# muzishen/IMAGDressing

Hardware: AMD Instinct MI355X
Metric: 512x512 50-step images/sec (whole node) (higher is better)
Workload: dtype bf16

## Files before the change

imagdressing_amd/csrc/conv_gemm.hip:

```cpp
#include "gemm_common.h"

namespace {

template <int BM, int BN, int BK, int WAVES_M> struct TileCfg {
    static constexpr int STRIDE = BK * 2 + 16;
    static constexpr int MAIN = 2 * (BM + BN) * STRIDE;
    static constexpr int CLD = BN + 4;
    static constexpr int EROWS = BM / WAVES_M;
    static constexpr int EPI = EROWS * CLD * 4;
    static constexpr int LDS = MAIN > EPI ? MAIN : EPI;
};

template <bool F16, int BM, int BN, int BK, int WAVES_M, int WAVES_N, int DEPTH>
__global__ __launch_bounds__(WAVES_M * WAVES_N * 64, (WAVES_M * WAVES_N == 4) ? 2 : 1) void conv_gemm_kernel(const ConvGemmParams p) {
    constexpr int NT = WAVES_M * WAVES_N * 64;
    using E = El<F16>;
    using T = TileCfg<BM, BN, BK, WAVES_M>;
    constexpr int TM = BM / WAVES_M / 32;
    constexpr int TN = BN / WAVES_N / 32;
    constexpr int STRIDE = T::STRIDE;
    constexpr int VPR = BK / 8;
    constexpr int RSTEP = NT / VPR;
    constexpr int A_VECS = BM / RSTEP;
    constexpr int W_VECS = BN / RSTEP;
// ... 461 lines not shown
        const int nparts = splitk_stats_parts_of(p);
        if (nparts == 0) return imd_set_error("%s: gn_stats_out on a K-sliced problem that cannot produce the statistics", what);
        const int HW = p.Hout * p.Wout, B = p.M / HW, rpp = fs_rows_per_part(B, HW, p.N);
        if (h) hipLaunchKernelGGL(splitk_finish_stats_kernel<true>, dim3((unsigned)nparts, (unsigned)B), dim3(FS_THREADS), 0, s, p, rpp, nparts);
        else hipLaunchKernelGGL(splitk_finish_stats_kernel<false>, dim3((unsigned)nparts, (unsigned)B), dim3(FS_THREADS), 0, s, p, rpp, nparts);
        return imd_check_launch(what);
    }
    const long chunks = (long)p.M * ((p.N + 7) / 8);
    long blocks = (chunks + 255) / 256;
    if (blocks > 2048) blocks = 2048;
    if (h) hipLaunchKernelGGL(splitk_finish_kernel<true>, dim3((unsigned)blocks), dim3(256), 0, s, p);
    else hipLaunchKernelGGL(splitk_finish_kernel<false>, dim3((unsigned)blocks), dim3(256), 0, s, p);
    return imd_check_launch(what);
}

template <bool F16, int BM, int BN, int BK, int WM, int WN, int DEPTH = 2>
int launch_cfg(const ConvGemmParams& p, hipStream_t s) {
    static_assert(DEPTH == 2 || DEPTH == 4, "pipeline depth");
    constexpr int lds = TileCfg<BM, BN, BK, WM>::LDS;
    auto kern = conv_gemm_kernel<F16, BM, BN, BK, WM, WN, DEPTH>;
    if (int rc_attr = imd_lds_attr(reinterpret_cast<const void*>(kern), lds, "conv_gemm")) return rc_attr;
    const long mt = (p.M + BM - 1) / BM, nt = (p.N + BN - 1) / BN;
    hipLaunchKernelGGL(kern, dim3((unsigned)(mt * nt), (unsigned)p.split_k), dim3(WM * WN * 64), lds, s, p);
    int rc = imd_check_launch("conv_gemm");
    if (rc || p.split_k <= 1 || p.splitk_counters != nullptr) return rc;
    return launch_splitk_finish(p, s, "conv_gemm split-K finish");
}

int tile_dims(int cfg, int* bm, int* bn) {
    switch (cfg) {
        case 0: *bm = 128; *bn = 128; return 0;
        case 1: *bm = 128; *bn = 64; return 0;
        case 2: *bm = 64; *bn = 64; return 0;
        case 4: case 5: case 8: case 29: *bm = 128; *bn = 128; return 0;
        case 3: case 7: *bm = 64; *bn = 64; return 0;
        case 6: *bm = 64; *bn = 320; return 0;
        case 9: case 21: case 30: case 31: *bm = 256; *bn = 128; return 0;
        case 32: *bm = 192; *bn = 128; return 0;
        case 22: *bm = 128; *bn = 160; return 0;
        case 23: *bm = 256; *bn = 160; return 0;
        case 24: *bm = 512; *bn = 64; return 0;
        case 10: case 16: *bm = 256; *bn = 256; return 0;
        case 17: case 18: case 19: case 20: case 25: case 26: case 27: case 28: *bm = 128; *bn = 128; return 0;
        case 11: *bm = 128; *bn = 320; return 0;
        default: return 1;
    }
}

}

int g_gemm_flags = 23;

int imd_gemm_pick_order(const ConvGemmParams& p, int n_tiles) {
    const double a_bytes = (double)p.x_bytes, w_bytes = (double)p.w_bytes / (p.split_k > 1 ? p.split_k : 1);
    const double a_split = a_bytes / (p.split_k > 1 && p.taps == 1 ? p.split_k : 1);
    const double cost_m = a_split + 8.0 * w_bytes;
    const double cost_n = (n_tiles < 8 ? n_tiles : 8) * a_split + w_bytes;
    return cost_m <= cost_n ? 4 : 8;
}

int imd_conv_gemm_stats_parts_of(const ConvGemmParams& p_in, int cfg) {
    ConvGemmParams p = p_in;
    if (p.split_k < 1) p.split_k = 1;
    if (cfg < 0) cfg = imd_conv_gemm_choose_cfg(p.M, p.N);
    if (p.split_k > 1) {
        if (cfg == 21 || cfg == 22 || cfg == 23 || cfg == 24 || cfg == 29 || (cfg >= 17 && cfg <= 20) || (cfg >= 25 && cfg <= 28) || (cfg >= 30 && cfg <= 32)) p.splitk_counters = nullptr;
        return splitk_stats_parts_of(p);
    }
    if (cfg == 22 || cfg == 23) return imd_conv_patch3_stats_parts_of(p, cfg == 23 ? 8 : 4);
    if (cfg == 5 || cfg == 29) return imd_conv_patch_stats_parts_of(p);
    if (cfg == 0 || cfg == 1 || cfg == 2 || cfg == 3 || cfg == 4 || cfg == 7) {
        int bm = 0, bn = 0;
        tile_dims(cfg, &bm, &bn);
        const int HW = p.Hout * p.Wout, G = p.gn_stats_groups;
        if (p.out_f32 || p.mode != OUT_ROWMAJOR || p.act == ACT_GEGLU || G <= 0 || G > 64 || p.N % G || (p.N / G) < 8 || (p.N % 4) || HW <= 0 || HW % bm || p.M % HW) return 0;
        return (HW / bm) * ((p.N + bn - 1) / bn);
    }
    return 0;
}

bool imd_row_linear_gn_in_supported_of(const ConvGemmParams& p, int cfg) {
    if (p.gn_in_partial == nullptr) return true;
    ConvGemmParams q = p;
    q.split_k = 1;
    switch (cfg) {
        case 12: return imd_row_linear_supported(q) && gn_in_ok(q, 320, 128);
        case 13: return imd_row_linear_k640_supported(q) && gn_in_ok(q, 640, 128);
        case 14: return imd_row_linear_k1280_supported(q) && gn_in_ok(q, 1280, 64);
        default: return false;
    }
}

bool imd_conv_gemm_gn_out_supported_of(const ConvGemmParams& p_in, int cfg) {
    ConvGemmParams p = p_in;
    (void)cfg;
    p.splitk_counters = nullptr;
    return splitk_gn_out_supported(p);
}

int imd_conv_gemm_choose_cfg(int M, int N) {
    const long b128 = (long)((M + 127) / 128) * ((N + 127) / 128);
    if (b128 < 96) return 2;
    if (N <= 64) return 1;
// ... 29 lines not shown
    if (p.M <= 0 || p.N <= 0 || p.K <= 0) return imd_set_error("conv_gemm: empty problem M=%d N=%d K=%d", p.M, p.N, p.K);
    if ((p.K % 8) || (p.Cin % 8) || (p.x_pix_stride % 8))
        return imd_set_error("conv_gemm: K (%d), Cin (%d) and pixel stride (%d) must be multiples of 8", p.K, p.Cin, p.x_pix_stride);
    if (p.N % 4) return imd_set_error("conv_gemm: N (%d) must be a multiple of 4", p.N);
    if (p.taps != 1 && p.taps != 9) return imd_set_error("conv_gemm: taps must be 1 or 9 (got %d)", p.taps);
    if (p.K != p.taps * p.Cin) return imd_set_error("conv_gemm: K (%d) != taps*Cin (%d)", p.K, p.taps * p.Cin);
    if (p.mode == OUT_HEADS && (p.hD % 8)) return imd_set_error("conv_gemm: head dim (%d) must be a multiple of 8", p.hD);
    if (p.act == ACT_GEGLU && (p.N % 8)) return imd_set_error("conv_gemm: GEGLU needs N %% 8 == 0");
    if (!imd_conv_gemm_fill_extents(p)) return imd_set_error("conv_gemm: operand larger than 4 GiB");
    if (cfg < 0) cfg = imd_conv_gemm_choose_cfg(p.M, p.N);
    if (p.split_k < 1) p.split_k = 1;
    const unsigned tag = (unsigned)p_in.flags & IMD_TUNING_TAG_MASK;
    if (tag != 0 && tag != (unsigned)IMD_TUNING_PER_CALL)
        return imd_set_error("conv_gemm: flags = 0x%x on entry is neither 0 nor IMD_TUNING_PER_CALL | bits (an uninitialised parameter block?)", (unsigned)p_in.flags);
    const int gf = (tag == (unsigned)IMD_TUNING_PER_CALL) ? ((p_in.flags & 31) | (g_gemm_flags & ~31)) : g_gemm_flags;
    {
        const int bk = (cfg == 4) ? 32 : 64;
        p.flags = 0;
        const bool big_map = p.taps == 9 && p.Wout >= 32;
        if ((gf & 1) && big_map && (p.Cin % bk) == 0) p.flags |= 1;
        if ((gf & 2) && big_map) p.flags |= 2;
    }
    if (gf & 4) {
        int bm = 128, bn = 128;
        tile_dims(cfg, &bm, &bn);
        p.flags |= imd_gemm_pick_order(p, (p.N + bn - 1) / bn);
        p.flags |= gf & 16;
    }
#ifdef IMD_ABLATIONS
    p.flags |= gf & 224;
#endif
    if (p.split_k <= 1) p.splitk_counters = nullptr;
    if (p.gn_stats_out != nullptr && imd_conv_gemm_stats_parts_of(p, cfg) == 0)
        return imd_set_error("conv_gemm: gn_stats_out needs tile config 5 / 22 / 23 / 29 or a register-staged tile (0..4, 7) with H W %% its rows == 0, without K slices, or any K-sliced launch with a separate finish; a row-major 16-bit "
                             "output and 1 <= groups <= 64 with N %% groups == 0 and N / groups >= 8 (got cfg=%d split_k=%d groups=%d N=%d); ask "
                             "imd_conv_gemm_stats_parts() first", cfg, p.split_k, p.gn_stats_groups, p.N);
    if (p.gn_out_gamma != nullptr && !imd_conv_gemm_gn_out_supported_of(p, cfg))
        return imd_set_error("conv_gemm: gn_out_* needs K slices with a separate finish launch, a row-major 16-bit output without residual / activation / scale / "
                             "gn_stats_out, 4 | N / groups and H W N / groups <= %d (got cfg=%d split_k=%d groups=%d N=%d); ask imd_conv_gemm_gn_out_supported() first",
                             4 * FG_THREADS * FG_MAXU, cfg, p.split_k, p.gn_out_groups, p.N);
    if (p.gn_out_gamma != nullptr) p.splitk_counters = nullptr;
    if (p.splitk_counters != nullptr) {
        int bm = 128, bn = 128;
        if (cfg == 5) { bm = 128; bn = 128; } else tile_dims(cfg, &bm, &bn);
        const long tiles = (cfg == 5) ? (long)(p.M / (p.Hout * p.Wout)) * ((p.Hout + 7) / 8) * ((p.Wout + 15) / 16) * ((p.N + 127) / 128)
                                      : (long)((p.M + bm - 1) / bm) * ((p.N + bn - 1) / bn);
        if (tiles > IMD_SPLITK_COUNTERS || (size_t)p.M * p.N * 4 >= 0x80000000ull) p.splitk_counters = nullptr;
    }
    if (p.split_k > 1) {
        if (p.mode == OUT_HEADS || p.act == ACT_GEGLU) return imd_set_error("conv_gemm: split-K supports row-major epilogues only");
        if (!p.splitk_ws) return imd_set_error("conv_gemm: split_k = %d needs a workspace", p.split_k);
    }
    if (p.dtype != IMD_DTYPE_BF16 && p.dtype != IMD_DTYPE_F16) return imd_set_error("conv_gemm: unknown dtype %d", p.dtype);
    if ((p.gn_a != nullptr) != (p.gn_b != nullptr)) return imd_set_error("conv_gemm: gn_a and gn_b must be given together");
    if (p.gn_a != nullptr && cfg != 5) return imd_set_error("conv_gemm: the fused GroupNorm prologue needs tile config 5 (got %d)", cfg);
    if (p.res_rows != 0 && cfg != 12)
        return imd_set_error("conv_gemm: a periodic residual (res_rows = %d) exists in the K = 320 row-resident projection only (tile config 12, got %d)", p.res_rows, cfg);
    if (p.gn_in_partial != nullptr && !imd_row_linear_gn_in_supported_of(p, cfg))
        return imd_set_error("conv_gemm: gn_in_* (GroupNorm of the input rows) exists in the row-resident projections only (tile configs 12 / 13 / 14 with H W a multiple of "
                             "their row block; got cfg=%d K=%d HW=%d): ask imd_row_linear_gn_in_supported() first", cfg, p.K, p.Hout * p.Wout);
    const bool h = p.dtype == IMD_DTYPE_F16;
    switch (cfg) {
        case 0: return h ? launch_cfg<true, 128, 128, 64, 2, 2>(p, s) : launch_cfg<false, 128, 128, 64, 2, 2>(p, s);
        case 1: return h ? launch_cfg<true, 128, 64, 64, 2, 2>(p, s) : launch_cfg<false, 128, 64, 64, 2, 2>(p, s);
        case 2: return h ? launch_cfg<true, 64, 64, 64, 2, 2>(p, s) : launch_cfg<false, 64, 64, 64, 2, 2>(p, s);
        case 3: return h ? launch_cfg<true, 64, 64, 64, 2, 2, 4>(p, s) : launch_cfg<false, 64, 64, 64, 2, 2, 4>(p, s);
        case 4: return h ? launch_cfg<true, 128, 128, 32, 2, 2>(p, s) : launch_cfg<false, 128, 128, 32, 2, 2>(p, s);
        case 6: return h ? launch_cfg<true, 64, 320, 32, 2, 2>(p, s) : launch_cfg<false, 64, 320, 32, 2, 2>(p, s);
        case 7: return h ? launch_cfg<true, 64, 64, 32, 2, 2, 4>(p, s) : launch_cfg<false, 64, 64, 32, 2, 2, 4>(p, s);
        case 8: return h ? launch_cfg<true, 128, 128, 32, 2, 2, 4>(p, s) : launch_cfg<false, 128, 128, 32, 2, 2, 4>(p, s);
        case 9: return h ? launch_cfg<true, 256, 128, 32, 4, 2>(p, s) : launch_cfg<false, 256, 128, 32, 4, 2>(p, s);
        case 10: return h ? launch_cfg<true, 256, 256, 32, 4, 2>(p, s) : launch_cfg<false, 256, 256, 32, 4, 2>(p, s);
        case 11: return h ? launch_cfg<true, 128, 320, 64, 4, 2>(p, s) : launch_cfg<false, 128, 320, 64, 4, 2>(p, s);
        case 5: {
            int rc = imd_launch_conv_patch(p, s);
            if (rc || p.split_k <= 1 || p.splitk_counters != nullptr) return rc;
            return launch_splitk_finish(p, s, "conv_patch split-K finish");
        }
        case 29: {
            p.splitk_counters = nullptr;
            int rc = imd_launch_conv_patch64(p, s);
            if (rc || p.split_k <= 1) return rc;
            return launch_splitk_finish(p, s, "conv_patch split-K finish");
        }
        case 21: {
            p.splitk_counters = nullptr;
            int rc = imd_launch_conv_patch2(p, s);
            if (rc || p.split_k <= 1) return rc;
            return launch_splitk_finish(p, s, "conv_patch2 split-K finish");
        }
        case 22: case 23: {
            int rc = cfg == 22 ? imd_launch_conv_patch3(p, s) : imd_launch_conv_patch4(p, s);
            if (rc || p.split_k <= 1) return rc;
            p.splitk_counters = nullptr;
            return launch_splitk_finish(p, s, "conv_patch3 split-K finish");
        }
        case 25: case 26: case 27: case 28: {
            if ((cfg == 26 || cfg == 28) != (p.taps == 9)) return imd_set_error("conv_gemm: tile config %d does not take taps = %d", cfg, p.taps);
            p.splitk_counters = nullptr;
            int rc = imd_launch_gemm_dma128(p, cfg >= 27 ? 13 : 12, s);
            if (rc || p.split_k <= 1) return rc;
            return launch_splitk_finish(p, s, "gemm_dma128 split-K finish");
        }
        case 24: {
            p.splitk_counters = nullptr;
            if (p.split_k <= 1) return imd_set_error("conv_gemm: tile config 24 writes K-slice slabs only (split_k >= 2)");
            int rc = imd_launch_conv_img(p, s);
            if (rc) return rc;
            return launch_splitk_finish(p, s, "conv_img split-K finish");
        }
        case 30: case 31: case 32: {
// ... 21 lines not shown
```

imagdressing_amd/csrc/conv_patch.hip:

```cpp
#include <type_traits>

#include "gemm_common.h"
#include "lds_dma.h"

namespace {

constexpr int TH = 8, TW = 16;
constexpr int PW = TW + 2, PH = TH + 2;
constexpr int NPIX = PH * PW;
constexpr int CK = 32;
constexpr int RSTR = CK * 2 + 16;
constexpr int BN = 128;
constexpr int A_BYTES = NPIX * RSTR;
constexpr int W_BYTES = BN * RSTR;
constexpr int MAIN_LDS = 2 * A_BYTES + 2 * W_BYTES;
constexpr int CLD = BN + 4;
constexpr int EROWS = 64;
constexpr int EPI_LDS = EROWS * CLD * 4;
constexpr int PATCH_LDS = MAIN_LDS > EPI_LDS ? MAIN_LDS : EPI_LDS;
constexpr int A_VECS = (NPIX * (CK / 8) + 255) / 256;
__device__ constexpr unsigned char kColPix[32] = {0, 1, 2, 3, 8, 9, 10, 11, 12, 13, 14, 15, 4, 5, 6, 7,
                                                  30, 31, 16, 17, 22, 23, 24, 25, 26, 27, 28, 29, 18, 19, 20, 21};
constexpr int W_VECS = BN * (CK / 8) / 256;

constexpr int AB_D = 12 * 1024, WB_D = 8 * 1024, NWR_D = 3;
constexpr int PATCH_DMA_LDS = 2 * AB_D + NWR_D * WB_D;
static_assert(PATCH_DMA_LDS >= EPI_LDS, "the epilogue tile must fit the main-loop LDS");
template <int CKD> struct PD {
    static constexpr int RB = CKD * 2, LPR = RB / 16;
    static constexpr int APIECES = (NPIX * RB + 1023) / 1024;
    static constexpr int APW = (APIECES + 3) / 4;
    static constexpr int AB = APW * 4 * 1024;
    static constexpr int WPW = BN * RB / 1024 / 4;
    static constexpr int WB = WPW * 4 * 1024;
    static constexpr int NWR = CKD == 32 ? 3 : 2;
    static constexpr int LDS = 2 * AB + NWR * WB;
    static_assert(LDS >= EPI_LDS, "the epilogue tile must fit the main-loop LDS");
    static __device__ __forceinline__ int swz(int r) { return CKD == 32 ? (r >> 2) & 3 : (r >> 1) & 7; }
};

template <bool F16, bool DMA, int CKD = 32>
__global__ __launch_bounds__(256, CKD == 32 ? 3 : 2) void conv3x3_patch_kernel(const ConvGemmParams p) {
    static_assert(CKD == 32 || DMA, "64-channel chunks exist for the LDS-DMA form only");
    using G = PD<CKD>;
    using E = El<F16>;
    extern __shared__ __attribute__((aligned(16))) char smem[];
    char* const Abuf = smem;
    char* const Wbuf = smem + 2 * A_BYTES;

    const int tid = threadIdx.x;
    const int lane = tid & 63;
    const int wave = tid >> 6;
    const int wm0 = (wave >> 1) * 64;
    const int wn0 = (wave & 1) * 64;
    const int hi = lane >> 5, col = lane & 31;
    const int cpix = kColPix[col];

    const int H = p.Hout, W = p.Wout;
    const int tiles_x = (W + TW - 1) / TW, tiles_y = (H + TH - 1) / TH;
    const int n_tiles = (p.N + BN - 1) / BN;
    int bid, tile_n;
    xcd_tile_order(p.flags, (int)(gridDim.x / n_tiles), n_tiles, bid, tile_n);
    const int tile_id = bid * n_tiles + tile_n;
    const int tx = bid % tiles_x; bid /= tiles_x;
    const int ty = bid % tiles_y;
    const int b = bid / tiles_y;
    const int y0 = ty * TH, x0 = tx * TW, n0 = tile_n * BN;

    const int nchunks = p.Cin / CKD;
    const int split = blockIdx.y;
    const int per = (nchunks + p.split_k - 1) / p.split_k;
    const int c_begin = split * per;
#ifdef PATCH_T_NOLOOP
    const int c_end = c_begin;
#else
    const int c_end = min(nchunks, c_begin + per);
// ... 82 lines not shown

    int a_frag[2];
#pragma unroll
    for (int bb = 0; bb < 2; ++bb) {
        const int q = wm0 + bb * 32 + cpix;
        a_frag[bb] = ((q / TW) * PW + (q % TW)) * RSTR + hi * 16;
    }
    const int w_frag = (wn0 + col) * RSTR + hi * 16;
    const bool wave_live = n0 + wn0 < p.N;

    if constexpr (DMA) {
        const int wv = __builtin_amdgcn_readfirstlane(wave);
        const uint32_t smem_base = (uint32_t)(uintptr_t)smem;
        const v4i_t dx = raw_rsrc(p.x, p.x_bytes), dw = raw_rsrc(p.w, p.w_bytes);
        constexpr uint32_t FAR = 0x80000000u;
        uint32_t acur[G::APW], wcur[G::WPW];
        uint32_t adst[G::APW], wdst[G::WPW];
#pragma unroll
        for (int i = 0; i < G::APW; ++i) {
            const int slot = (wv * G::APW + i) * 64 + lane, pp = slot / G::LPR, piece = (slot % G::LPR) ^ G::swz(pp);
            acur[i] = FAR;
            if (pp < NPIX) {
                const int iy = y0 - 1 + pp / PW, ix = x0 - 1 + pp % PW;
                if ((unsigned)iy < (unsigned)H && (unsigned)ix < (unsigned)W) {
                    const int sy = p.ups ? (iy >> 1) : iy, sx = p.ups ? (ix >> 1) : ix;
                    acur[i] = (uint32_t)(((b * p.Hin + sy) * p.Win + sx) * p.x_pix_stride + piece * 8 + c_begin * CKD) * 2u;
                }
            }
            adst[i] = smem_base + (uint32_t)((wv * G::APW + i) * 1024);
        }
#pragma unroll
        for (int i = 0; i < G::WPW; ++i) {
            const int slot = (wv * G::WPW + i) * 64 + lane, row = slot / G::LPR, piece = (slot % G::LPR) ^ G::swz(row);
            wcur[i] = (n0 + row < p.N) ? (uint32_t)(((size_t)(n0 + row) * p.K + piece * 8 + c_begin * CKD) * 2) : FAR;
            wdst[i] = smem_base + (uint32_t)(2 * G::AB + (wv * G::WPW + i) * 1024);
        }
        const uint32_t w_tap = (uint32_t)(p.Cin * 2), w_chunk = (uint32_t)(CKD * 2) - 8u * w_tap;
        auto dma_patch = [&](auto buf_c) __attribute__((always_inline)) {
#pragma unroll
            for (int i = 0; i < G::APW; ++i) {
                asm volatile("s_add_u32 m0, %1, %3\n\ts_nop 0\n\tbuffer_load_dwordx4 %0, %2, 0 offen lds"
                             : : "v"(acur[i]), "s"(adst[i]), "s"(dx), "n"(decltype(buf_c)::value * G::AB) : "memory", "scc");
                acur[i] += (uint32_t)(CKD * 2);
            }
        };
        auto dma_w = [&](auto ring_c, auto cross_c) __attribute__((always_inline)) {
#pragma unroll
            for (int i = 0; i < G::WPW; ++i) {
                asm volatile("s_add_u32 m0, %1, %3\n\ts_nop 0\n\tbuffer_load_dwordx4 %0, %2, 0 offen lds"
                             : : "v"(wcur[i]), "s"(wdst[i]), "s"(dw), "n"(decltype(ring_c)::value * G::WB) : "memory", "scc");
                wcur[i] += decltype(cross_c)::value ? w_chunk : w_tap;
            }
        };
        int w_fr[2], xa[9][2];
#pragma unroll
        for (int a = 0; a < 2; ++a) {
            const int row = wn0 + a * 32 + col;
            w_fr[a] = row * G::RB + ((hi ^ G::swz(row)) << 4);
        }
#pragma unroll
        for (int bb = 0; bb < 2; ++bb) {
            const int q = wm0 + bb * 32 + cpix, r0 = (q / TW) * PW + (q % TW);
#pragma unroll
            for (int t = 0; t < 9; ++t) {
                const int rw = r0 + (t / 3) * PW + (t % 3);
                xa[t][bb] = rw * G::RB + ((hi ^ G::swz(rw)) << 4);
            }
        }
        const bool live = __builtin_amdgcn_readfirstlane((int)(n0 + (wv & 1) * 64 < p.N)) != 0;
        const std::integral_constant<int, 0> i0{}; const std::integral_constant<int, 1> i1{}; const std::integral_constant<int, 2> i2{};
        if (total > 0) {
            dma_patch(i0);
            dma_w(i0, std::false_type{});
            if (G::NWR == 3) dma_w(i1, std::false_type{});
        }
        dma_wait();
        __syncthreads();
        auto chunk = [&](auto ab_c) __attribute__((always_inline)) {
            constexpr int AB = decltype(ab_c)::value;
            const char* As = smem + AB * G::AB;
#pragma unroll
            for (int t = 0; t < 9; ++t) {
                constexpr int LEAD = G::NWR - 1;
                const int cur = G::NWR == 3 ? t % 3 : (9 * AB + t) % 2;
                if (G::NWR == 3) {
                    if (t % 3 == 0) dma_w(i2, std::false_type{});
                    else if (t % 3 == 1) dma_w(i0, std::false_type{});
                    else dma_w(i1, std::false_type{});
                } else {
                    if (((9 * AB + t) & 1) == 0) dma_w(i1, std::false_type{}); else dma_w(i0, std::false_type{});
                }
                if (t == 8 - LEAD) {
#pragma unroll
                    for (int i = 0; i < G::WPW; ++i) wcur[i] += w_chunk - w_tap;
                }
                if (t == 5) dma_patch(std::integral_constant<int, AB ^ 1>{});
                if (live) {
                    const char* Ws = smem + 2 * G::AB + cur * G::WB;
#pragma unroll
                    for (int k2 = 0; k2 < CKD / 32; ++k2) {
                        uint4 wf[2][2], xf[2][2];
#pragma unroll
                        for (int kk = 0; kk < 2; ++kk) {
#pragma unroll
                            for (int a = 0; a < 2; ++a) wf[kk][a] = *reinterpret_cast<const uint4*>(Ws + (w_fr[a] ^ ((2 * k2 + kk) * 32)));
#pragma unroll
                            for (int bb = 0; bb < 2; ++bb) xf[kk][bb] = *reinterpret_cast<const uint4*>(As + (xa[t][bb] ^ ((2 * k2 + kk) * 32)));
                        }
#pragma unroll
                        for (int kk = 0; kk < 2; ++kk)
#pragma unroll
                            for (int a = 0; a < 2; ++a)
#pragma unroll
                                for (int bb = 0; bb < 2; ++bb) acc[a][bb] = E::mfma(wf[kk][a], xf[kk][bb], acc[a][bb]);
                    }
                }
                if (G::NWR == 3) { if (t == 5 || t == 6) dma_wait_keep_n<G::WPW + G::APW>(); else dma_wait_keep_n<G::WPW>(); }
                else { if (t == 5) dma_wait_keep_n<G::APW>(); else dma_wait(); }
                __syncthreads();
            }
        };
        const int nch = c_end - c_begin;
        int cc = 0;
#pragma unroll 1
        for (; cc + 2 <= nch; cc += 2) { chunk(i0); chunk(i1); }
// ... 171 lines not shown

}

int imd_conv_patch_stats_parts_of(const ConvGemmParams& p) {
    if (!imd_conv_patch_supported(p) || p.split_k > 1 || p.out_f32 || p.gn_stats_groups <= 0 || p.gn_stats_groups > 64 ||
        p.N % p.gn_stats_groups || (p.N / p.gn_stats_groups) < 8)
        return 0;
    return ((p.Hout + TH - 1) / TH) * ((p.Wout + TW - 1) / TW) * ((p.N + BN - 1) / BN);
}

bool imd_conv_patch_supported(const ConvGemmParams& p) {
    const bool geom = p.ups ? (p.Hout == 2 * p.Hin && p.Wout == 2 * p.Win && p.gn_a == nullptr && !(g_gemm_flags & 512))
                            : (p.Hin == p.Hout && p.Win == p.Wout);
    return p.taps == 9 && p.stride == 1 && !p.pad_br_only && geom && p.Hout >= TH && p.Wout >= TW && (p.Cin % CK) == 0 &&
           p.mode == OUT_ROWMAJOR && p.act != ACT_GEGLU;
}

bool imd_conv_patch64_supported(const ConvGemmParams& p) {
    return imd_conv_patch_supported(p) && (p.Cin % 64) == 0 && p.gn_a == nullptr && !(g_gemm_flags & 512) && p.x_bytes < 0x80000000u && p.w_bytes < 0x80000000u;
}

int imd_launch_conv_patch64(const ConvGemmParams& p, hipStream_t s) {
    if (!imd_conv_patch64_supported(p)) return imd_set_error("conv_patch (128-byte rows): unsupported problem (needs 3x3 stride 1, H >= 8, W >= 16, Cin %% 64 == 0, operands < 2 GiB, no fused GroupNorm)");
    const bool h = p.dtype == IMD_DTYPE_F16;
    typedef void (*kern_t)(const ConvGemmParams);
    const kern_t kern = h ? conv3x3_patch_kernel<true, true, 64> : conv3x3_patch_kernel<false, true, 64>;
    if (int rc_attr = imd_lds_attr(reinterpret_cast<const void*>(kern), PD<64>::LDS, "conv_patch")) return rc_attr;
    const int B = p.M / (p.Hout * p.Wout);
    const long blocks = (long)B * ((p.Hout + TH - 1) / TH) * ((p.Wout + TW - 1) / TW) * ((p.N + BN - 1) / BN);
    hipLaunchKernelGGL(kern, dim3((unsigned)blocks, (unsigned)p.split_k), dim3(256), PD<64>::LDS, s, p);
    return imd_check_launch("conv_patch (128-byte rows)");
}

int imd_launch_conv_patch(const ConvGemmParams& p, hipStream_t s) {
    if (!imd_conv_patch_supported(p)) return imd_set_error("conv_patch: unsupported geometry (needs 3x3 stride 1, H >= 8, W >= 16, Cin %% 32 == 0)");
    const bool h = p.dtype == IMD_DTYPE_F16;
    const bool dma = p.gn_a == nullptr && !(g_gemm_flags & 512) && (p.ups || (p.x_bytes < 0x80000000u && p.w_bytes < 0x80000000u));
    if (p.ups && (p.x_bytes >= 0x80000000u || p.w_bytes >= 0x80000000u)) return imd_set_error("conv_patch: fused upsample needs operands < 2 GiB");
    typedef void (*kern_t)(const ConvGemmParams);
    const kern_t kern = dma ? (h ? conv3x3_patch_kernel<true, true> : conv3x3_patch_kernel<false, true>)
                            : (h ? conv3x3_patch_kernel<true, false> : conv3x3_patch_kernel<false, false>);
    const int lds = dma ? PATCH_DMA_LDS : PATCH_LDS;
    if (int rc_attr = imd_lds_attr(reinterpret_cast<const void*>(kern), lds, "conv_patch")) return rc_attr;
    const int B = p.M / (p.Hout * p.Wout);
    const long blocks = (long)B * ((p.Hout + TH - 1) / TH) * ((p.Wout + TW - 1) / TW) * ((p.N + BN - 1) / BN);
    hipLaunchKernelGGL(kern, dim3((unsigned)blocks, (unsigned)p.split_k), dim3(256), lds, s, p);
    return imd_check_launch("conv_patch");
}
```

imagdressing_amd/csrc/imd_kernels.h:

```cpp
#pragma once
#include <hip/hip_runtime.h>
#include <stdint.h>

#include "../../include/imagdressing_hip.h"

typedef uint16_t bf16_t;
typedef imd_heads_dest HeadsDest;
typedef imd_conv_gemm_params ConvGemmParams;
typedef imd_attn_params AttnParams;
typedef imd_groupnorm_params GroupNormParams;
typedef imd_layernorm_params LayerNormParams;
typedef imd_ddim_params DdimParams;

enum { ACT_NONE = IMD_ACT_NONE, ACT_SILU = IMD_ACT_SILU, ACT_GEGLU = IMD_ACT_GEGLU, ACT_GELU = IMD_ACT_GELU, ACT_QUICK_GELU = IMD_ACT_QUICK_GELU };
enum { OUT_ROWMAJOR = IMD_OUT_ROWMAJOR, OUT_HEADS = IMD_OUT_HEADS };

int imd_set_error(const char* fmt, ...);
int imd_check_launch(const char* what);
int imd_lds_attr(const void* kern, int bytes, const char* what);
int imd_cu_count8();

int imd_conv_gemm_choose_cfg(int M, int N);
int imd_conv_gemm_choose_split(int M, int N, int K, int cfg);
int imd_launch_conv_gemm(const ConvGemmParams& p, int cfg, hipStream_t s);
bool imd_conv_gemm_fill_extents(ConvGemmParams& p);
bool imd_conv_patch_supported(const ConvGemmParams& p);
bool imd_conv_patch2_supported(const ConvGemmParams& p);
int imd_launch_conv_patch2(const ConvGemmParams& p, hipStream_t s);
bool imd_conv_patch3_supported(const ConvGemmParams& p);
int imd_launch_conv_patch3(const ConvGemmParams& p, hipStream_t s);
bool imd_conv_patch4_supported(const ConvGemmParams& p);
int imd_launch_conv_patch4(const ConvGemmParams& p, hipStream_t s);
int imd_conv_patch3_stats_parts_of(const ConvGemmParams& p, int nw);
bool imd_conv_patch64_supported(const ConvGemmParams& p);
int imd_launch_conv_patch64(const ConvGemmParams& p, hipStream_t s);
bool imd_conv_img_supported(const ConvGemmParams& p);
int imd_launch_conv_img(const ConvGemmParams& p, hipStream_t s);
int imd_conv_patch_stats_parts_of(const ConvGemmParams& p);
int imd_conv_gemm_stats_parts_of(const ConvGemmParams& p, int cfg);
bool imd_conv_gemm_gn_out_supported_of(const ConvGemmParams& p, int cfg);
bool imd_row_linear_gn_in_supported_of(const ConvGemmParams& p, int cfg);
int imd_launch_conv_patch(const ConvGemmParams& p, hipStream_t s);
bool imd_row_linear_supported(const ConvGemmParams& p);
int imd_launch_row_linear(const ConvGemmParams& p, int ln, float ln_eps, hipStream_t s);
bool imd_row_linear_k640_supported(const ConvGemmParams& p);
int imd_launch_row_linear_k640(const ConvGemmParams& p, int ln, float ln_eps, hipStream_t s);
bool imd_row_linear_k1280_supported(const ConvGemmParams& p);
int imd_launch_row_linear_k1280(const ConvGemmParams& p, int ln, float ln_eps, hipStream_t s);
bool imd_row_qkv_supported(const ConvGemmParams& p);
int imd_launch_row_qkv(const ConvGemmParams& p, int ln, float ln_eps, hipStream_t s);
bool imd_gemm_dma_supported(const ConvGemmParams& p);
int imd_launch_gemm_dma(const ConvGemmParams& p, hipStream_t s);
int imd_launch_gemm_dma128(const ConvGemmParams& p, int stages, hipStream_t s);
int imd_launch_gemm_dma256(const ConvGemmParams& p, int form, hipStream_t s);
bool imd_conv_dma_supported(const ConvGemmParams& p);
int imd_launch_ff_geglu(const imd_ff_params& p, hipStream_t s);
int imd_launch_attention(const AttnParams& p, hipStream_t s);
int imd_launch_attention_d40(const AttnParams& p, int variant, hipStream_t s);
int imd_launch_attention_fp8(const AttnParams& p, int eq, int ek, int ev, hipStream_t s);
int imd_launch_attn_quantize_fp8(const bf16_t* src, unsigned char* dst, int kind, long rows_or_groups, int LP, int exp2_scale,
                                 float pad_val, int dtype, hipStream_t s);
extern int g_attn_qw40;
extern int g_attn_xcd;
#ifdef IMD_ATTN_SWEEP
extern int g_attn_v80, g_attn_v160;
#endif
extern int g_gemm_flags;
int imd_attn_dpk(int D);
int imd_attn_dpv(int D);
int imd_launch_groupnorm(const GroupNormParams& p, hipStream_t s);
int imd_launch_groupnorm_coeffs(const GroupNormParams& p, float* ca, float* cb, hipStream_t s);
int imd_groupnorm_parts_of(int B, int HW, int C);
int imd_launch_concat2_gn_stats(const bf16_t* a, int Ca, const bf16_t* b, int Cb, const bf16_t* b_add, bf16_t* out, int B, int HW, int b_B, int G,
                                float* partial, int dtype, hipStream_t s);
int imd_launch_layernorm(const LayerNormParams& p, hipStream_t s);
// ... 12 lines not shown
```

imagdressing_amd/ops.py:

```python
from __future__ import annotations

import functools
import ctypes as C
from typing import Dict, Optional, Sequence, Tuple

import torch

from . import _lib as L

ACT_NONE, ACT_SILU, ACT_GEGLU, ACT_GELU, ACT_QUICK_GELU = 0, 1, 2, 3, 4
bf16 = torch.bfloat16
f16 = torch.float16
DTYPE_CODE = {torch.bfloat16: 0, torch.float16: 1}


def _code(t: torch.Tensor, name: str = "tensor") -> int:
    try:
        return DTYPE_CODE[t.dtype]
    except KeyError:
        raise L.ImdError(f"{name}: expected a bfloat16 or float16 tensor, got {t.dtype}") from None


try:
    _raw_stream, _cur_dev = torch._C._cuda_getCurrentRawStream, torch._C._cuda_getDevice
# ... 83 lines not shown
def _count(kind: str, flops: float):
    c = FLOP_COUNTER
    if c is not None:
        c[kind] = c.get(kind, 0.0) + float(flops)


def attn_padded_dims(D: int) -> Tuple[int, int]:
    a, b = C.c_int(), C.c_int()
    L.check(L.load().imd_attn_padded_dims(D, C.byref(a), C.byref(b)))
    return a.value, b.value


def pad64(n: int) -> int:
    return (n + 63) // 64 * 64


PATCH_CONV = True
PATCH_MIN_W = 32
SPLITK_IN_KERNEL = False
FUSED_FF = True
FUSED_FF_MIN_ROWS = 24576
import os as _os
FUSED_GN_STATS = _os.environ.get("IMD_FUSED_GN_STATS", "1") != "0"
CFG_PAIR_DEDUP = _os.environ.get("IMD_CFG_PAIR_DEDUP", "1") != "0"
FUSED_GN_CONV = _os.environ.get("IMD_FUSED_GN_CONV", "0") == "1"
FUSED_GN_FINISH = _os.environ.get("IMD_FUSED_GN_FINISH", "0") == "1"
FUSED_GN_PROJ = _os.environ.get("IMD_FUSED_GN_PROJ", "1") != "0"
FUSED_CONCAT_STATS = _os.environ.get("IMD_FUSED_CONCAT_STATS", "1") != "0"
PERIODIC_RES = _os.environ.get("IMD_PERIODIC_RES", "1") != "0"
GENERIC_GN_STATS = _os.environ.get("IMD_GENERIC_GN_STATS", "0") == "1"
TEMB_TABLE = _os.environ.get("IMD_TEMB_TABLE", "1") != "0"
FUSED_GN_PROJ_CFGS = tuple(int(c) for c in _os.environ.get("IMD_FUSED_GN_PROJ_CFGS", "12,13,14").split(",") if c)
CFG_PAIR_ATTN = _os.environ.get("IMD_CFG_PAIR_ATTN", "1") != "0"
FUSED_LN = True
GEMM_TRACE = None
GEMM_EVENT_HOOK = None
_GEMM_TABLE = None
_CFG_DECISIONS: Dict[Tuple, Tuple[int, int]] = {}

TUNING_PER_CALL = 0x5A000000
ATTN_VARIANT_MAX = 13


import contextvars

_TUNING = contextvars.ContextVar("imd_tuning_scope", default=None)


class tuning_scope:

    def __init__(self, attn_variant=None, attn_xcd=None, gemm_flags=None):
        self.new = dict(attn_variant=attn_variant, attn_xcd=attn_xcd, gemm_flags=gemm_flags)

    def __enter__(self):
        merged = dict(_TUNING.get() or {})
        merged.update({k: v for k, v in self.new.items() if v is not None})
        self.token = _TUNING.set(merged if any(v is not None for v in merged.values()) else None)
        return self

    def __exit__(self, *exc):
        _TUNING.reset(self.token)
        return False


def _gemm_call_flags() -> int:
    t = _TUNING.get()
    if t is None or t.get("gemm_flags") is None:
        return 0
    return TUNING_PER_CALL | (int(t["gemm_flags"]) & 31)


def _attn_call_flags() -> int:
    t = _TUNING.get()
    if t is None or (t.get("attn_variant") is None and t.get("attn_xcd") is None):
        return 0
    v = int(t.get("attn_variant") or 0)
    if not 0 <= v <= ATTN_VARIANT_MAX:
        raise L.ImdError(f"tuning_scope: attention variant {v} out of range 0..{ATTN_VARIANT_MAX} (imd_set_tuning(0, .) of the product build)")
    if t.get("attn_xcd") is None:
        xcd = bool(L.load().imd_get_tuning(1))
    else:
        xcd = bool(t["attn_xcd"])
    return TUNING_PER_CALL | v | (0 if xcd else 256)


def _gemm_table() -> dict:
    global _GEMM_TABLE
    if _GEMM_TABLE is None:
        import json
        import os
        path = os.environ.get("IMD_GEMM_TUNING") or os.path.join(os.path.dirname(os.path.abspath(__file__)), "gemm_tuning.json")
        try:
            with open(path) as f:
                _GEMM_TABLE = json.load(f).get("shapes", {})
        except FileNotFoundError:
            _GEMM_TABLE = {}
    return _GEMM_TABLE


def conv_gemm(
    x: torch.Tensor, w: torch.Tensor, *, M: int, N: int, Cin: int, taps: int = 1,
    Hin: int = 1, Win: int = 1, Hout: int = 1, Wout: int = 1, stride: int = 1, ups: bool = False,
    x_pix_stride: Optional[int] = None, out: Optional[torch.Tensor] = None, out_ld: Optional[int] = None,
    bias: Optional[torch.Tensor] = None, rowvec: Optional[torch.Tensor] = None, rowvec_stride: int = 0,
    rowvec_off: int = 0, res: Optional[torch.Tensor] = None, res_ld: Optional[int] = None, out_scale: float = 1.0,
    act: int = ACT_NONE, out_f32: bool = False,
    heads: Optional[dict] = None, cfg: int = -1, split_k: int = 0,
    gn: Optional[tuple] = None, pad_br_only: bool = False, ln_eps: Optional[float] = None, gn_stats_groups: int = 0,
    gn_out: Optional[tuple] = None, gn_in: Optional[tuple] = None,
) -> Optional[torch.Tensor]:
    ensure_device(x.device)
    K = taps * Cin
    p = L.ConvGemmParams()
    p.flags = _gemm_call_flags()
    dt = x.dtype
    p.dtype = _code(x, "x")
    p.x = _dev(x, dt, "x")
    p.w = _dev(w, dt, "w")
    if w.numel() != N * K:
        raise L.ImdError(f"conv_gemm: weight has {w.numel()} elements, expected N*K = {N}*{K}")
    p.M, p.N, p.K = M, N, K
    p.Cin, p.taps, p.Hin, p.Win, p.Hout, p.Wout, p.stride, p.ups = Cin, taps, Hin, Win, Hout, Wout, stride, int(ups)
    p.x_pix_stride = Cin if x_pix_stride is None else x_pix_stride
    p.bias = _opt(bias, torch.float32, "bias")
    p.rowvec = _opt(rowvec, torch.float32, "rowvec")
    if rowvec is not None and rowvec_off:
        if rowvec_off % 4:
            raise L.ImdError("conv_gemm: rowvec_off must be a multiple of 4")
        p.rowvec = p.rowvec + 4 * rowvec_off
    p.rowvec_stride = rowvec_stride
# ... 10 lines not shown
    p.out_f32 = int(out_f32)
    if heads is not None:
        p.mode = 1
        p.hC, p.hH, p.hD = heads["C"], heads["H"], heads["D"]
        for i, (t, kind, DP, Ltok, scale) in enumerate(heads["dests"]):
            p.hd[i].ptr = None if t is None else _dev(t, dt, f"heads[{i}]")
            p.hd[i].kind, p.hd[i].DP, p.hd[i].L, p.hd[i].scale = kind, DP, Ltok, scale
        p.out = None
        p.out_ld = 0
    else:
        p.mode = 0
        n_out = N // 2 if act == ACT_GEGLU else N
        if out is None:
            out = torch.empty((M, n_out), dtype=torch.float32 if out_f32 else dt, device=x.device)
        p.out = _dev(out, torch.float32 if out_f32 else dt, "out")
        p.out_ld = n_out if out_ld is None else out_ld
    _count("gemm_conv", 2.0 * M * N * K)
    lib = L.load()
    if gn is not None:
        p.gn_a, p.gn_b, p.gn_silu = _dev(gn[0], torch.float32, "gn_a"), _dev(gn[1], torch.float32, "gn_b"), int(gn[2])
        if cfg == -1:
            cfg = 5
    if ln_eps is not None:
        if res_rows:
            if K == 320 and res_rows % 128 == 0 and PERIODIC_RES:
                p.res_rows = res_rows
            else:
                res = repeat_batch(res.reshape(res_rows, N), M // res_rows)
                p.res = _dev(res, dt, "res")
        p.split_k = 1
        L.check(lib.imd_row_linear(C.byref(p), 1, float(ln_eps), _stream()))
        return out
    splittable = heads is None and act != ACT_GEGLU
    if GEMM_TRACE is not None:
        GEMM_TRACE.append(dict(M=M, N=N, K=K, Cin=Cin, taps=taps, Hin=Hin, Win=Win, Hout=Hout, Wout=Wout, stride=stride,
                               ups=int(ups), splittable=splittable, dtype=str(dt)))
    dkey = None
    if cfg == -1 and split_k == 0 and GEMM_TRACE is None:
        hk = None if heads is None else (heads["C"], heads["H"], heads["D"], tuple((t is None, kind, DP, Ltok) for t, kind, DP, Ltok, _ in heads["dests"]))
        dkey = (M, N, K, Cin, taps, stride, int(ups), Hin, Win, Hout, Wout, p.x_pix_stride, p.res_ld, p.out_ld, act, int(out_f32), int(pad_br_only), p.dtype,
                rowvec is None, res is None, bias is None, hk, PATCH_CONV, id(_GEMM_TABLE))
        hit = _CFG_DECISIONS.get(dkey)
        if hit is not None:
            cfg, split_k = hit
    if cfg == -1 and split_k == 0:
        key = f"{M},{N},{K},{taps},{stride},{int(ups)}"
        ent = (_gemm_table().get(f"{key}|{Hout}x{Wout}") if taps == 9 else None) or _gemm_table().get(key)
        if ent is not None:
            if splittable:
                cfg, split_k = ent["cfg"], ent["split"]
            else:
                cfg, split_k = ent["cfg_nosplit"], 1
            if cfg == 5 and not lib.imd_conv_patch_supported(C.byref(p)):
                cfg, split_k = -1, 0
            if cfg in (12, 13, 14, 15) and not lib.imd_row_linear_supported(C.byref(p)):
                cfg, split_k = -1, 0
            if cfg in (16, 17, 19, 25, 27, 30, 31, 32) and not lib.imd_gemm_dma_supported(C.byref(p)):
                cfg, split_k = -1, 0
            if (cfg in (18, 20) and (taps != 9 or Cin % 32 or stride not in (1, 2) or gn is not None)) or \
                    (cfg in (26, 28) and (taps != 9 or Cin % 64 or stride not in (1, 2) or gn is not None)):
                cfg, split_k = -1, 0
            if cfg == 21 and not lib.imd_conv_patch2_supported(C.byref(p)):
                cfg, split_k = -1, 0
            if cfg == 22 and not lib.imd_conv_patch3_supported(C.byref(p)):
                cfg, split_k = -1, 0
            if cfg == 23 and not lib.imd_conv_patch4_supported(C.byref(p)):
# ... 20 lines not shown
        gi_gamma, gi_beta, gi_eps, gi_silu, gi_groups = gn_in
        st = getattr(x, "_imd_gn_stats", None)
        fused = False
        if FUSED_GN_PROJ and cfg in FUSED_GN_PROJ_CFGS and st is not None and st[2] == gi_groups and FUSED_GN_STATS and st[0].shape[0] * Hout * Wout == M:
            p.gn_in_partial, p.gn_in_nparts, p.gn_in_groups = st[0].data_ptr(), st[1], int(gi_groups)
            p.gn_in_gamma, p.gn_in_beta = _dev(gi_gamma, torch.float32, "gn_in gamma"), _dev(gi_beta, torch.float32, "gn_in beta")
            p.gn_in_eps, p.gn_in_silu = float(gi_eps), int(bool(gi_silu))
            fused = bool(lib.imd_row_linear_gn_in_supported(C.byref(p), cfg))
            if not fused:
                p.gn_in_partial = None
                p.gn_in_nparts = p.gn_in_groups = 0
        if not fused:
            xv = x.view(M // (Hout * Wout), Hout * Wout, Cin)
            if st is not None:
                xv._imd_gn_stats = st
            xn = group_norm(xv, gi_gamma, gi_beta, groups=gi_groups, eps=gi_eps, silu=gi_silu)
            p.x = _dev(xn, dt, "x")
    if split_k > 1:
        p.splitk_ws = splitk_workspace(split_k * M * N, x.device).data_ptr()
        if SPLITK_IN_KERNEL:
            p.splitk_counters = splitk_counters(x.device).data_ptr()
    if gn_out is not None and FUSED_GN_FINISH and split_k > 1 and heads is None and not out_f32 and act == ACT_NONE and res is None and out_scale == 1.0:
        g_gamma, g_beta, g_eps, g_silu, g_groups = gn_out
        p.gn_out_gamma, p.gn_out_beta = _dev(g_gamma, torch.float32, "gn_out gamma"), _dev(g_beta, torch.float32, "gn_out beta")
        p.gn_out_eps, p.gn_out_silu, p.gn_out_groups = float(g_eps), int(bool(g_silu)), int(g_groups)
        if lib.imd_conv_gemm_gn_out_supported(C.byref(p)):
            p.splitk_counters = None
            gn_stats_groups = 0
            L.check(lib.imd_conv_gemm(C.byref(p), cfg, _stream()))
            out._imd_gn_applied = True
            return out
        p.gn_out_gamma = p.gn_out_beta = None
        p.gn_out_groups = 0
    stats = None
    if gn_stats_groups and FUSED_GN_STATS and heads is None and not out_f32 and act != ACT_GEGLU and \
            (cfg in (5, 22, 23, 29) or split_k > 1 or (GENERIC_GN_STATS and cfg in (-1, 0, 1, 2, 3, 4, 7))):
        p.gn_stats_groups = gn_stats_groups
        nparts = lib.imd_conv_gemm_stats_parts(C.byref(p), cfg)
        if nparts > 0:
            Bimg = M // (Hout * Wout)
            stats = (torch.empty((Bimg, nparts, gn_stats_groups, 2), dtype=torch.float32, device=x.device), nparts, gn_stats_groups)
            p.gn_stats_out = stats[0].data_ptr()
        else:
            p.gn_stats_groups = 0
    if GEMM_EVENT_HOOK is not None:
        e0, e1 = torch.cuda.Event(enable_timing=True), torch.cuda.Event(enable_timing=True)
        e0.record()
        L.check(lib.imd_conv_gemm(C.byref(p), cfg, _stream()))
        e1.record()
        GEMM_EVENT_HOOK.setdefault((f"{M},{N},{K},{taps},{stride},{int(ups)}|{Hout}x{Wout}", cfg, split_k), []).append((e0, e1))
    else:
        L.check(lib.imd_conv_gemm(C.byref(p), cfg, _stream()))
    if stats is not None:
        out._imd_gn_stats = stats
    return out


_splitk_ws: Dict[Tuple, torch.Tensor] = {}


_splitk_cnt: Dict[Tuple, torch.Tensor] = {}


def splitk_counters(device) -> torch.Tensor:
    key = (str(device), _stream())
    t = _splitk_cnt.get(key)
    if t is None:
        t = torch.zeros(16384, dtype=torch.int32, device=device)
        _splitk_cnt[key] = t
# ... 448 lines not shown
```

Before: 6.949.

## Add tile-packed weight layout for 3x3 patch conv kernel

Adds a new config 33 that runs the LDS-DMA 3x3 patch conv kernel on weights repacked once on the host side into per-tile, per-chunk, per-tap contiguous blocks, with the LDS swizzle already applied. Each wave's weight DMA then reads a contiguous slab instead of strided rows, and per-chunk pointer fixups go away. It is enabled by default for auto-selected config 5 convs with N >= 128. Packed copies are cached on the weight tensor, at the cost of extra memory and a fallback when packing would happen during graph capture.

```diff
diff --git a/imagdressing_amd/csrc/conv_gemm.hip b/imagdressing_amd/csrc/conv_gemm.hip
--- a/imagdressing_amd/csrc/conv_gemm.hip
+++ b/imagdressing_amd/csrc/conv_gemm.hip
@@ -517,7 +517,7 @@
         case 0: *bm = 128; *bn = 128; return 0;
         case 1: *bm = 128; *bn = 64; return 0;
         case 2: *bm = 64; *bn = 64; return 0;
-        case 4: case 5: case 8: case 29: *bm = 128; *bn = 128; return 0;
+        case 4: case 5: case 8: case 29: case 33: *bm = 128; *bn = 128; return 0;
         case 3: case 7: *bm = 64; *bn = 64; return 0;
         case 6: *bm = 64; *bn = 320; return 0;
         case 9: case 21: case 30: case 31: *bm = 256; *bn = 128; return 0;
@@ -553,7 +553,7 @@
         return splitk_stats_parts_of(p);
     }
     if (cfg == 22 || cfg == 23) return imd_conv_patch3_stats_parts_of(p, cfg == 23 ? 8 : 4);
-    if (cfg == 5 || cfg == 29) return imd_conv_patch_stats_parts_of(p);
+    if (cfg == 5 || cfg == 29 || cfg == 33) return imd_conv_patch_stats_parts_of(p);
     if (cfg == 0 || cfg == 1 || cfg == 2 || cfg == 3 || cfg == 4 || cfg == 7) {
         int bm = 0, bn = 0;
         tile_dims(cfg, &bm, &bn);
@@ -649,7 +649,7 @@
 #endif
     if (p.split_k <= 1) p.splitk_counters = nullptr;
     if (p.gn_stats_out != nullptr && imd_conv_gemm_stats_parts_of(p, cfg) == 0)
-        return imd_set_error("conv_gemm: gn_stats_out needs tile config 5 / 22 / 23 / 29 or a register-staged tile (0..4, 7) with H W %% its rows == 0, without K slices, or any K-sliced launch with a separate finish; a row-major 16-bit "
+        return imd_set_error("conv_gemm: gn_stats_out needs tile config 5 / 22 / 23 / 29 / 33 or a register-staged tile (0..4, 7) with H W %% its rows == 0, without K slices, or any K-sliced launch with a separate finish; a row-major 16-bit "
                              "output and 1 <= groups <= 64 with N %% groups == 0 and N / groups >= 8 (got cfg=%d split_k=%d groups=%d N=%d); ask "
                              "imd_conv_gemm_stats_parts() first", cfg, p.split_k, p.gn_stats_groups, p.N);
     if (p.gn_out_gamma != nullptr && !imd_conv_gemm_gn_out_supported_of(p, cfg))
@@ -659,8 +659,8 @@
     if (p.gn_out_gamma != nullptr) p.splitk_counters = nullptr;
     if (p.splitk_counters != nullptr) {
         int bm = 128, bn = 128;
-        if (cfg == 5) { bm = 128; bn = 128; } else tile_dims(cfg, &bm, &bn);
-        const long tiles = (cfg == 5) ? (long)(p.M / (p.Hout * p.Wout)) * ((p.Hout + 7) / 8) * ((p.Wout + 15) / 16) * ((p.N + 127) / 128)
+        if (cfg == 5 || cfg == 33) { bm = 128; bn = 128; } else tile_dims(cfg, &bm, &bn);
+        const long tiles = (cfg == 5 || cfg == 33) ? (long)(p.M / (p.Hout * p.Wout)) * ((p.Hout + 7) / 8) * ((p.Wout + 15) / 16) * ((p.N + 127) / 128)
                                       : (long)((p.M + bm - 1) / bm) * ((p.N + bn - 1) / bn);
         if (tiles > IMD_SPLITK_COUNTERS || (size_t)p.M * p.N * 4 >= 0x80000000ull) p.splitk_counters = nullptr;
     }
@@ -694,6 +694,11 @@
             if (rc || p.split_k <= 1 || p.splitk_counters != nullptr) return rc;
             return launch_splitk_finish(p, s, "conv_patch split-K finish");
         }
+        case 33: {
+            int rc = imd_launch_conv_patch_packed(p, s);
+            if (rc || p.split_k <= 1 || p.splitk_counters != nullptr) return rc;
+            return launch_splitk_finish(p, s, "conv_patch split-K finish");
+        }
         case 29: {
             p.splitk_counters = nullptr;
             int rc = imd_launch_conv_patch64(p, s);
diff --git a/imagdressing_amd/csrc/conv_patch.hip b/imagdressing_amd/csrc/conv_patch.hip
--- a/imagdressing_amd/csrc/conv_patch.hip
+++ b/imagdressing_amd/csrc/conv_patch.hip
@@ -39,9 +39,10 @@
     static __device__ __forceinline__ int swz(int r) { return CKD == 32 ? (r >> 2) & 3 : (r >> 1) & 7; }
 };
 
-template <bool F16, bool DMA, int CKD = 32>
+template <bool F16, bool DMA, int CKD = 32, bool PACKW = false>
 __global__ __launch_bounds__(256, CKD == 32 ? 3 : 2) void conv3x3_patch_kernel(const ConvGemmParams p) {
     static_assert(CKD == 32 || DMA, "64-channel chunks exist for the LDS-DMA form only");
+    static_assert(!PACKW || (DMA && CKD == 32), "tile-packed weights exist for the 32-channel LDS-DMA form only");
     using G = PD<CKD>;
     using E = El<F16>;
     extern __shared__ __attribute__((aligned(16))) char smem[];
@@ -190,10 +191,11 @@
 #pragma unroll
         for (int i = 0; i < G::WPW; ++i) {
             const int slot = (wv * G::WPW + i) * 64 + lane, row = slot / G::LPR, piece = (slot % G::LPR) ^ G::swz(row);
-            wcur[i] = (n0 + row < p.N) ? (uint32_t)(((size_t)(n0 + row) * p.K + piece * 8 + c_begin * CKD) * 2) : FAR;
+            if constexpr (PACKW) wcur[i] = (uint32_t)((tile_n * nchunks + c_begin) * 9 * G::WB + slot * 16);
+            else wcur[i] = (n0 + row < p.N) ? (uint32_t)(((size_t)(n0 + row) * p.K + piece * 8 + c_begin * CKD) * 2) : FAR;
             wdst[i] = smem_base + (uint32_t)(2 * G::AB + (wv * G::WPW + i) * 1024);
         }
-        const uint32_t w_tap = (uint32_t)(p.Cin * 2), w_chunk = (uint32_t)(CKD * 2) - 8u * w_tap;
+        const uint32_t w_tap = PACKW ? (uint32_t)G::WB : (uint32_t)(p.Cin * 2), w_chunk = PACKW ? (uint32_t)G::WB : (uint32_t)(CKD * 2) - 8u * w_tap;
         auto dma_patch = [&](auto buf_c) __attribute__((always_inline)) {
 #pragma unroll
             for (int i = 0; i < G::APW; ++i) {
@@ -248,7 +250,7 @@
                 } else {
                     if (((9 * AB + t) & 1) == 0) dma_w(i1, std::false_type{}); else dma_w(i0, std::false_type{});
                 }
-                if (t == 8 - LEAD) {
+                if (!PACKW && t == 8 - LEAD) {
 #pragma unroll
                     for (int i = 0; i < G::WPW; ++i) wcur[i] += w_chunk - w_tap;
                 }
@@ -486,6 +488,22 @@
     return imd_check_launch("conv_patch (128-byte rows)");
 }
 
+int imd_launch_conv_patch_packed(const ConvGemmParams& p_in, hipStream_t s) {
+    ConvGemmParams p = p_in;
+    const size_t wb = (size_t)((p.N + BN - 1) / BN * BN) * p.K * 2;
+    p.w_bytes = wb < 0x80000000ull ? (uint32_t)wb : 0x80000000u;
+    if (!imd_conv_patch_supported(p) || p.gn_a != nullptr || (g_gemm_flags & 512) || p.x_bytes >= 0x80000000u || p.w_bytes >= 0x80000000u)
+        return imd_set_error("conv_patch (tile-packed weights): unsupported problem (needs 3x3 stride 1, H >= 8, W >= 16, Cin %% 32 == 0, operands < 2 GiB, no fused GroupNorm, the LDS-DMA form)");
+    const bool h = p.dtype == IMD_DTYPE_F16;
+    typedef void (*kern_t)(const ConvGemmParams);
+    const kern_t kern = h ? conv3x3_patch_kernel<true, true, 32, true> : conv3x3_patch_kernel<false, true, 32, true>;
+    if (int rc_attr = imd_lds_attr(reinterpret_cast<const void*>(kern), PATCH_DMA_LDS, "conv_patch")) return rc_attr;
+    const int B = p.M / (p.Hout * p.Wout);
+    const long blocks = (long)B * ((p.Hout + TH - 1) / TH) * ((p.Wout + TW - 1) / TW) * ((p.N + BN - 1) / BN);
+    hipLaunchKernelGGL(kern, dim3((unsigned)blocks, (unsigned)p.split_k), dim3(256), PATCH_DMA_LDS, s, p);
+    return imd_check_launch("conv_patch (tile-packed weights)");
+}
+
 int imd_launch_conv_patch(const ConvGemmParams& p, hipStream_t s) {
     if (!imd_conv_patch_supported(p)) return imd_set_error("conv_patch: unsupported geometry (needs 3x3 stride 1, H >= 8, W >= 16, Cin %% 32 == 0)");
     const bool h = p.dtype == IMD_DTYPE_F16;
diff --git a/imagdressing_amd/csrc/imd_kernels.h b/imagdressing_amd/csrc/imd_kernels.h
--- a/imagdressing_amd/csrc/imd_kernels.h
+++ b/imagdressing_amd/csrc/imd_kernels.h
@@ -41,6 +41,7 @@
 bool imd_conv_gemm_gn_out_supported_of(const ConvGemmParams& p, int cfg);
 bool imd_row_linear_gn_in_supported_of(const ConvGemmParams& p, int cfg);
 int imd_launch_conv_patch(const ConvGemmParams& p, hipStream_t s);
+int imd_launch_conv_patch_packed(const ConvGemmParams& p, hipStream_t s);
 bool imd_row_linear_supported(const ConvGemmParams& p);
 int imd_launch_row_linear(const ConvGemmParams& p, int ln, float ln_eps, hipStream_t s);
 bool imd_row_linear_k640_supported(const ConvGemmParams& p);
diff --git a/imagdressing_amd/ops.py b/imagdressing_amd/ops.py
--- a/imagdressing_amd/ops.py
+++ b/imagdressing_amd/ops.py
@@ -139,6 +139,8 @@
 TEMB_TABLE = _os.environ.get("IMD_TEMB_TABLE", "1") != "0"
 FUSED_GN_PROJ_CFGS = tuple(int(c) for c in _os.environ.get("IMD_FUSED_GN_PROJ_CFGS", "12,13,14").split(",") if c)
 CFG_PAIR_ATTN = _os.environ.get("IMD_CFG_PAIR_ATTN", "1") != "0"
+PACKED_CONV_W = _os.environ.get("IMD_PACKED_CONV_W", "1") != "0"
+PACKED_CONV_W_BYTES = 0
 FUSED_LN = True
 GEMM_TRACE = None
 GEMM_EVENT_HOOK = None
@@ -203,6 +205,40 @@
         except FileNotFoundError:
             _GEMM_TABLE = {}
     return _GEMM_TABLE
+
+
+def pack_conv_patch_weights(w: torch.Tensor, N: int, Cin: int) -> torch.Tensor:
+    if Cin % 32 or w.numel() != N * 9 * Cin:
+        raise L.ImdError(f"pack_conv_patch_weights: needs Cin % 32 == 0 and N x 9 Cin elements (N={N}, Cin={Cin}, numel={w.numel()})")
+    NT, nch = (N + 127) // 128, Cin // 32
+    wp = torch.zeros((NT * 128, 9 * Cin), dtype=w.dtype, device=w.device)
+    wp[:N] = w.reshape(N, 9 * Cin)
+    v = wp.view(NT, 128, 9, nch, 4, 8).permute(0, 3, 2, 1, 4, 5)
+    return torch.gather(v, 4, _packw_index(w.device).expand(NT, nch, 9, 128, 4, 8)).reshape(-1)
+
+
+def unpack_conv_patch_weights(wp: torch.Tensor, N: int, Cin: int) -> torch.Tensor:
+    NT, nch = (N + 127) // 128, Cin // 32
+    v = torch.gather(wp.view(NT, nch, 9, 128, 4, 8), 4, _packw_index(wp.device).expand(NT, nch, 9, 128, 4, 8))
+    return v.permute(0, 3, 2, 1, 4, 5).reshape(NT * 128, 9 * Cin)[:N]
+
+
+def _packw_index(device) -> torch.Tensor:
+    r, q = torch.arange(128, device=device).view(128, 1), torch.arange(4, device=device).view(1, 4)
+    return (q ^ ((r >> 2) & 3)).view(1, 1, 1, 128, 4, 1)
+
+
+def _packed_conv_w(w: torch.Tensor, N: int, Cin: int) -> Optional[torch.Tensor]:
+    global PACKED_CONV_W_BYTES
+    hit = getattr(w, "_imd_packw", None)
+    if hit is not None and hit[0] == w._version:
+        return hit[1]
+    if torch.cuda.is_current_stream_capturing():
+        return None
+    wp = pack_conv_patch_weights(w, N, Cin)
+    w._imd_packw = (w._version, wp)
+    PACKED_CONV_W_BYTES += wp.numel() * wp.element_size()
+    return wp
 
 
 def conv_gemm(
@@ -279,6 +315,7 @@
         L.check(lib.imd_row_linear(C.byref(p), 1, float(ln_eps), _stream()))
         return out
     splittable = heads is None and act != ACT_GEGLU
+    auto_cfg = cfg == -1
     if GEMM_TRACE is not None:
         GEMM_TRACE.append(dict(M=M, N=N, K=K, Cin=Cin, taps=taps, Hin=Hin, Win=Win, Hout=Hout, Wout=Wout, stride=stride,
                                ups=int(ups), splittable=splittable, dtype=str(dt)))
@@ -365,9 +402,17 @@
             return out
         p.gn_out_gamma = p.gn_out_beta = None
         p.gn_out_groups = 0
+    if cfg == 33 or (cfg == 5 and auto_cfg and PACKED_CONV_W and gn is None and N >= 128 and x.numel() * x.element_size() < 0x80000000
+                     and (N + 127) // 128 * 128 * K * 2 < 0x80000000 and not (lib.imd_get_tuning(2) & 512)):
+        wp = _packed_conv_w(w, N, Cin)
+        if wp is not None:
+            cfg = 33
+            p.w = wp.data_ptr()
+        elif cfg == 33:
+            raise L.ImdError("conv_gemm: tile config 33 needs the packed weights, which cannot be made while a HIP graph is being captured")
     stats = None
     if gn_stats_groups and FUSED_GN_STATS and heads is None and not out_f32 and act != ACT_GEGLU and \
-            (cfg in (5, 22, 23, 29) or split_k > 1 or (GENERIC_GN_STATS and cfg in (-1, 0, 1, 2, 3, 4, 7))):
+            (cfg in (5, 22, 23, 29, 33) or split_k > 1 or (GENERIC_GN_STATS and cfg in (-1, 0, 1, 2, 3, 4, 7))):
         p.gn_stats_groups = gn_stats_groups
         nparts = lib.imd_conv_gemm_stats_parts(C.byref(p), cfg)
         if nparts > 0:
```

New measurement: 7.014, median of 6. About the same (+0.9%).
